# DanielTakeshi/gym-cloth

Hardware: AMD Instinct MI355X
Metric: cloth substeps/sec (25x25 grid, batched envs) (higher is better)
Workload: dtype f32

## Files before the change

### gym_cloth_amd/csrc/episode_loop.hpp

```cpp
#pragma once

#include "cloth_common.hpp"
#include "phase_strain.hpp"
#include "phase_collide.hpp"
#include "cloth_metrics.hpp"

namespace clothhip {

template <typename T, int NT, int PPT, int TAB, bool REST_REG, int FUSED, int NS = 0>
__global__ __launch_bounds__(NT, (Variant{(int)sizeof(T), NT, PPT, TAB, REST_REG}.waves_per_eu())) void k_run_schedule(StepArgs<T> A) {
    static_assert((NS == 0 || NS == 25 || NS == 50) && (NS == 0 || FUSED != 3), "grid-specialised builds exist for 25x25 and 50x50 (stepper_variants.hpp: CLOTH_SPEC_*)");
    static constexpr Variant V{(int)sizeof(T), NT, PPT, TAB, REST_REG};
    extern __shared__ __attribute__((aligned(16))) unsigned char smem[];
    const int e = blockIdx.x + A.e0;
    const int tid = threadIdx.x;
    const int lane = tid & 63;
    const FusedArgs<T> *const Fp = A.fz;
    constexpr bool fused = FUSED != 0;
    constexpr bool with_tier2 = FUSED == 2;
    constexpr bool RELAXED = FUSED == 3;
    ClothSchedule sc;
    if (!fused) {
        sc = A.sched[e];
        if (!sc.active || sc.n_total <= 0) {
            if (tid == 0) A.executed[e] = 0;
            return;
        }
    } else {
        sc.n_up_end = sc.n_uprest_end = sc.n_pull_end = sc.n_griprest_end = sc.n_total = 0;
        sc.break_on_tear = 1; sc.active = 1; sc._pad = 0;
        sc.dz_up = sc.dx_pull = sc.dy_pull = sc.dz_pull = 0.0;
    }
    const int P = NS > 0 ? spec_p(NS) : A.P, Ppad = NS > 0 ? spec_ppad(NS) : A.Ppad, HT = NS > 0 ? spec_ht(NS, V) : A.HT;
    constexpr bool LEAN64 = V.lean64();
    const LdsLayout lay = lds_layout(V, Ppad, KA_SPAD(&A), HT, KA_CELLCOPY(&A));
    Pt<T> *cur = reinterpret_cast<Pt<T> *>(smem + lay.cur);
    uint32_t *hkey = reinterpret_cast<uint32_t *>(smem + lay.hkey);
    uint32_t *hco = reinterpret_cast<uint32_t *>(smem + lay.hco);
    uint16_t *memb = reinterpret_cast<uint16_t *>(smem + lay.memb);
    uint16_t *slot = reinterpret_cast<uint16_t *>(smem + lay.slot);
    int *misc = reinterpret_cast<int *>(smem + lay.misc);
    uint16_t *olist = reinterpret_cast<uint16_t *>(smem + lay.olist);
    uint16_t *alist_end = olist + (Ppad - 1);
    Pt<T> *cpos = reinterpret_cast<Pt<T> *>(smem + lay.cpos);
    const T *g_rest = A.rest + (size_t)e * A.rest_stride;
    const WEnt<T> *wtab = reinterpret_cast<const WEnt<T> *>(smem + lay.wtab);
    auto rest_at = [&](uint32_t i) -> T { return V.table_in_lds() ? wtab[i].rest : g_rest[i]; };
    const int pm = NS > 0 ? (PH_HOOKE | PH_COLLIDE | PH_PLANE | PH_STRAIN) : A.phase_mask;

    T pvx[PPT], pvy[PPT], pvz[PPT];
    constexpr bool LEAN = V.lean();
    constexpr bool GT_REG = sizeof(T) == 4 && !LEAN;
    constexpr bool REST_R = V.rest_in_registers();
    uint32_t gt[GT_REG ? PPT : 1][HK_SLOTS];
    T rr[REST_R ? PPT : 1][HK_SLOTS];
    uint32_t vm[(LEAN && !LEAN64) ? PPT : 1];
    const uint4 *const lstc = reinterpret_cast<const uint4 *>(smem + lay.lstc);
    auto lean_rest64 = [&](int sl, const uint4 &lw) -> T {
        const uint32_t wsel = sl < 4 ? lw.y : (sl < 8 ? lw.z : lw.w);
        const uint32_t off = (wsel >> (8 * (sl & 3))) & 0xFFu;
        const double base = (double)(lean_bend(sl) ? A.pal_bend : (lean_shear(sl) ? A.pal_shear : A.pal_struct));
        return (T)__longlong_as_double(__double_as_longlong(base) + (long long)off);
    };
    (void)lean_rest64; (void)lstc;
    uint32_t rc[RELAXED ? PPT : 1];
    constexpr bool LEAN_NATIVE = LEAN && !LEAN64 && V.lean_native_gather();
    static_assert(!LEAN_NATIVE || (2 * NS <= V.cur_front_pad_records() && 2 * 27 <= V.cur_front_pad_records()), "the records in front of `cur` must cover the stencil's reach (two rows)");
    auto lean_entry = [&](int i, uint32_t vmq, int sl) -> uint32_t {
        const bool ok = ((vmq >> sl) & 1u) != 0u;
        return (uint32_t)(ok ? i + lean_off(sl, KA_N(&A)) : i) | (ok ? HK_VALID : 0u) | (sl < HK_SLOTS / 2 ? HK_ASB : 0u) |
               (lean_bend(sl) ? HK_BEND : 0u);
    };
    auto lean_rest = [&](int sl) -> T {
        if constexpr (NS > 0 && sizeof(T) == 4)
            return (T)(lean_bend(sl) ? spec_pal(NS, 2) : (lean_shear(sl) ? spec_pal(NS, 1) : spec_pal(NS, 0)));
        else return lean_bend(sl) ? A.pal_bend : (lean_shear(sl) ? A.pal_shear : A.pal_struct);
    };
    {
        const T *gp = A.pos + (size_t)e * 3 * Ppad, *gq = A.prev + (size_t)e * 3 * Ppad;
        const uint8_t *gc = A.cnt + (size_t)e * Ppad;
        if constexpr (V.cur_front_pad_records() > 0) {
            static_assert(V.cur_front_pad_records() <= NT, "one thread per record in front of `cur`");
            if (tid < V.cur_front_pad_records()) cur[tid - V.cur_front_pad_records()] = Pt<T>{(T)0, (T)0, (T)0, (T)0};
        }
        for (int i = tid; i < Ppad; i += NT)
            cur[i] = Pt<T>{gp[i], gp[Ppad + i], gp[2 * Ppad + i], w_make<T>(gc[i])};
#pragma unroll
        for (int q = 0; q < PPT; q++) {
            const int i = tid + q * NT;
            const bool ok = i < P;
            pvx[q] = ok ? gq[i] : (T)0; pvy[q] = ok ? gq[Ppad + i] : (T)0; pvz[q] = ok ? gq[2 * Ppad + i] : (T)0;
            if (LEAN64) { }
            else if (LEAN) { const int r_ = i / KA_N(&A); vm[(LEAN && !LEAN64) ? q : 0] = ok ? lean_valid_mask(r_, i - r_ * KA_N(&A), KA_N(&A)) : 0u; if (RELAXED) rc[RELAXED ? q : 0] = (uint32_t)r_ | ((uint32_t)(i - r_ * KA_N(&A)) << 8); }
            else
#pragma unroll
            for (int sl = 0; sl < HK_SLOTS; sl++) {
                const uint32_t g0 = ok ? A.gather[sl * Ppad + i] : 0u;
                if (GT_REG) gt[GT_REG ? q : 0][sl] = g0;
                if (REST_R) rr[REST_R ? q : 0][sl] = g_rest[(g0 >> HK_POS_SHIFT) & HK_POS_MASK];
            }
        }
    }
    auto init_lds = [&](int tear_flag, const uint32_t *s_ent, const T *s_rest) {
        if (V.table_in_lds() && s_ent != nullptr) {
            WEnt<T> *d0 = reinterpret_cast<WEnt<T> *>(smem + lay.wtab);
            for (int i = tid; i < KA_SPAD(&A); i += NT) { WEnt<T> w_; w_.ab = s_ent[i]; w_.rest = s_rest[i]; d0[i] = w_; }
        }
        for (int h = tid; h < HT; h += NT) { hkey[h] = KEY_EMPTY; hco[h] = 0; }
        if (tid == 0) { misc[0] = tear_flag; misc[1] = 0; misc[2] = 0; misc[3] = 0; misc[4] = 0; misc[5] = 0; misc[6] = 0; misc[10] = 0x7fffffff; misc[11] = -1; misc[12] = 0; misc[13] = 0; misc[14] = 0; misc[20] = 0; misc[21] = 0; misc[22] = 0; misc[23] = 0; }
    };
    if (tid == 0) misc[15] = 0;
    init_lds(A.tear[e], A.wt_ent, g_rest);
    if (LEAN64) {
        uint4 *d_ = reinterpret_cast<uint4 *>(smem + lay.lstc);
        for (int i = tid; i < Ppad; i += NT) d_[i] = A.lstc[i];
    }
    uint16_t *pslot = reinterpret_cast<uint16_t *>(smem + lay.pslot);
    if (V.has_point_slots()) {
        for (int i = tid; i < Ppad; i += NT) {
            const int r_ = i / KA_N(&A);
            const uint32_t vmi = i < P ? lean_valid_mask(r_, i - r_ * KA_N(&A), KA_N(&A)) : 0u;
#pragma unroll
            for (int sl = 0; sl < HK_SLOTS / 2; sl++)
                pslot[sl * Ppad + i] = ((vmi >> sl) & 1u) ? (uint16_t)((A.gather[__popc(vmi & ((1u << sl) - 1u)) * Ppad + i] >> HK_POS_SHIFT) & HK_POS_MASK) : (uint16_t)0;
        }
    }
    __syncthreads();

    int st_windows = 0, st_passes = 0, st_commits = 0;
#ifdef CLOTHHIP_TPH_LDS
    const TphLds tph{reinterpret_cast<unsigned long long *>(smem + lay.tphs), tid == 0};
    if (tid < 12) tph.base[tid] = 0ull;
    unsigned long long tlast = 0, tstart = 0;
#else
    unsigned long long tph[12] = {0, 0, 0, 0, 0, 0, 0, 0, 0, 0, 0, 0}, tlast = 0, tstart = 0;
#endif
    asm volatile("s_memtime %0\n\ts_waitcnt lgkmcnt(0)" : "=s"(tstart)::"memory");
#ifdef CLOTHHIP_DIAG_PLACEMENT
    const unsigned long long diag_t0_ = __builtin_amdgcn_s_memrealtime();
#endif
#ifdef CLOTHHIP_PHASE_STAMPS
    const bool timing = (pm & PH_TIME) != 0;
#else
    constexpr bool timing = false;
#endif
#ifdef CLOTHHIP_SWEEP_STAMPS
    constexpr bool SWEEP_TIMED = true;
#else
    constexpr bool SWEEP_TIMED = false;
#endif
#if !defined(CLOTHHIP_SWEEP_STAMPS) && !defined(CLOTHHIP_CELL_COUNTERS)
    constexpr bool SWEEP_LEAN = true;
#else
    constexpr bool SWEEP_LEAN = false;
#endif
    constexpr bool SWEEP_AHEAD = V.sweep_read_ahead();
    (void)SWEEP_AHEAD;
#if defined(CLOTHHIP_PHASE_STAMPS) || defined(CLOTHHIP_CELL_COUNTERS)
    constexpr bool SWEEP_STATS = true;
#else
    constexpr bool SWEEP_STATS = false;
#endif
#define TSTAMP(slot_)                                                          \
    if (timing) {                                                              \
        unsigned long long tn_;                                                \
        __builtin_amdgcn_sched_barrier(0);                                     \
        asm volatile("s_memtime %0\n\ts_waitcnt lgkmcnt(0)" : "=s"(tn_)::"memory"); \
        __builtin_amdgcn_sched_barrier(0);                                     \
        tph[slot_] += tn_ - tlast; tlast = tn_;                                \
    }
    if (timing) { asm volatile("s_memtime %0\n\ts_waitcnt lgkmcnt(0)" : "=s"(tlast)::"memory"); }

    enum { OP_SCHED = 0, OP_ACTION, OP_RESET_COND, OP_RESET_PULL, OP_RESET_SETTLE, OP_RESET_END };
    EpState *const eps = reinterpret_cast<EpState *>(smem + lay.eps);
    auto account = [&](int op_, int n_sub) {
        const int cls = op_ == OP_ACTION ? 0 : ((op_ == OP_RESET_PULL || op_ == OP_RESET_COND) ? 1 : (op_ == OP_RESET_SETTLE ? 2 : 3));
        const uint64_t now_ = __builtin_amdgcn_s_memrealtime();
        eps->ticks[cls] += now_ - eps->t_mark; eps->t_mark = now_; eps->subs[cls] += (uint32_t)n_sub;
    };
    if (fused) {
        if (tid == 0) {
            eps->t_slot = 0; eps->rp = -1; eps->n_resets = 0; eps->chain_ok = 1; eps->rs_pulls = 0; eps->reset_mark = 0;
            eps->ep_steps = Fp->num_steps[e]; eps->ep_done = Fp->done[e] ? 1 : 0; eps->done_total = 0; eps->stop = 0;
            misc[7] = 0;
            eps->t_mark = __builtin_amdgcn_s_memrealtime();
            for (int q = 0; q < 4; q++) { eps->ticks[q] = 0; eps->subs[q] = 0; }
            eps->last_cov = __longlong_as_double(0x7ff8000000000000LL); eps->n_ran = 0;
            eps->swap = Fp->policy_arg != nullptr ? Fp->policy_arg[e] : 0; eps->choice = 0;
            if (Fp->resume != nullptr && Fp->resume[e].valid) {
                const EpResume *rs_ = Fp->resume + e;
                const EpState &o = rs_->eps;
                eps->rp = o.rp; eps->chain_ok = o.chain_ok; eps->rs_pulls = o.rs_pulls; eps->ep_steps = o.ep_steps;
                eps->ep_done = o.ep_done; eps->op = o.op; eps->n_grab = o.n_grab; eps->iters_pull = o.iters_pull;
                eps->decode_err = o.decode_err; eps->side = o.side; eps->pull = o.pull; eps->choice = o.choice; eps->swap = o.swap;
                eps->act[0] = o.act[0]; eps->act[1] = o.act[1]; eps->act[2] = o.act[2]; eps->act[3] = o.act[3];
                if (o.rp >= 0 && Fp->resets != nullptr) Fp->resets[(size_t)e * Fp->n_scripts] = rs_->rr;
                if constexpr (with_tier2)
                    if (Fp->expert != 0 && o.rp < 0 && rs_->it >= 0) { double *lp = Fp->labels + 4 * (size_t)e; for (int q = 0; q < 4; q++) lp[q] = Fp->resume_labelled ? rs_->label[q] : __longlong_as_double(-1LL); }
            }
        }
        __syncthreads();
    }
    int resume_it = -1, resume_done = 0;
    if (FUSED) {
        if (Fp->resume != nullptr && Fp->resume[e].valid) {
            const EpResume *rs_ = Fp->resume + e;
            resume_it = rs_->it; resume_done = rs_->done_partial;
            if (resume_it >= 0) sc = rs_->sc;
        }
        __syncthreads();
        if (tid == 0 && Fp->resume != nullptr) Fp->resume[e].valid = 0;
    }
    if (FUSED) {
        if (tid == 0) {
            eps->t_launch = __builtin_amdgcn_s_memrealtime();
            eps->t_deadline = Fp->budget_ticks != 0 ? eps->t_launch + Fp->budget_ticks : ~0ull;
        }
    }
    int done_nf = 0;
    for (;;) {
        bool do_run = true;
        const bool resumed_run = FUSED && resume_it >= 0;
        if (fused && resumed_run) {
            sc.n_up_end = __builtin_amdgcn_readfirstlane(sc.n_up_end);
            sc.n_uprest_end = __builtin_amdgcn_readfirstlane(sc.n_uprest_end);
            sc.n_pull_end = __builtin_amdgcn_readfirstlane(sc.n_pull_end);
            sc.n_griprest_end = __builtin_amdgcn_readfirstlane(sc.n_griprest_end);
            sc.n_total = __builtin_amdgcn_readfirstlane(sc.n_total);
            sc.break_on_tear = __builtin_amdgcn_readfirstlane(sc.break_on_tear);
        }
        if (fused && !resumed_run) {
#include "episode_plan.inc.hpp"
        }
        int done = resumed_run ? resume_done : 0;
        int it_next = -1;
        {
        auto uni = [](T v) -> T {
            if constexpr (sizeof(T) == 4) return __int_as_float(__builtin_amdgcn_readfirstlane(__float_as_int((float)v)));
            else return __hiloint2double(__builtin_amdgcn_readfirstlane(__double2hiint((double)v)), __builtin_amdgcn_readfirstlane(__double2loint((double)v)));
        };
        const T dz_up = uni((T)sc.dz_up), dxp = uni((T)sc.dx_pull), dyp = uni((T)sc.dy_pull), dzp = uni((T)sc.dz_pull);
        const bool sliced = FUSED && Fp->budget_ticks != 0 && Fp->resume != nullptr;
        const int n_up_end_ = __builtin_amdgcn_readfirstlane(sc.n_up_end);
        const int n_uprest_end_ = __builtin_amdgcn_readfirstlane(sc.n_uprest_end);
        const int n_pull_end_ = __builtin_amdgcn_readfirstlane(sc.n_pull_end);
        const int n_griprest_end_ = __builtin_amdgcn_readfirstlane(sc.n_griprest_end);
        const int n_total_ = __builtin_amdgcn_readfirstlane(sc.n_total);
        const int break_on_tear_ = __builtin_amdgcn_readfirstlane(sc.break_on_tear);
        const int it0_ = __builtin_amdgcn_readfirstlane(resumed_run ? resume_it : 0);
    const int tid_outer_ = tid;
#ifdef CLOTHHIP_CELL_COUNTERS
    bool frozen_prev_ = false; (void)frozen_prev_;
#endif
    for (int it = it0_; it < n_total_; it++) {
        int tid = tid_outer_;
        if (LEAN || sizeof(T) == 8 || NT >= 512) asm volatile("" : "+v"(tid));
        const int lane = tid & 63;
        KArgsC<T> *Ak_ = (KArgsC<T> *)__builtin_amdgcn_kernarg_segment_ptr();

#include "substep_pull.inc.hpp"
        TSTAMP(0)
#include "substep_hooke_verlet.inc.hpp"
        TSTAMP(1)
#include "substep_collision.inc.hpp"
#include "substep_plane.inc.hpp"
        if (FUSED && sliced) {
            if (tid == 0) misc[7] = (__builtin_amdgcn_s_memrealtime() >= eps->t_deadline) ? 1 : 0;
        }
        __syncthreads();

        TSTAMP(7)
#include "substep_strain.inc.hpp"
        if (timing) { asm volatile("s_memtime %0\n\ts_waitcnt lgkmcnt(0)" : "=s"(tlast)::"memory"); }
        done++;
        if (break_on_tear_ && misc[0]) break;
        if (FUSED && sliced && misc[7] && it + 1 < n_total_) { it_next = it + 1; break; }
    }
        }
        resume_it = -1;
        if (!fused) { done_nf = done; break; }
#include "episode_finish.inc.hpp"
    }
    const int done = fused ? eps->done_total : done_nf;

#undef TSTAMP
    {
        __syncthreads();
        T *gp = A.pos + (size_t)e * 3 * Ppad, *gq = A.prev + (size_t)e * 3 * Ppad;
        uint8_t *gc = A.cnt + (size_t)e * Ppad;
        for (int i = tid; i < Ppad; i += NT) {
            const Pt<T> c = cur[i];
            gp[i] = c.x; gp[Ppad + i] = c.y; gp[2 * Ppad + i] = c.z; gc[i] = (uint8_t)w_cnt(c.w);
        }
#pragma unroll
        for (int q = 0; q < PPT; q++) {
            const int i = tid + q * NT;
            if (i < P) { gq[i] = pvx[q]; gq[Ppad + i] = pvy[q]; gq[2 * Ppad + i] = pvz[q]; }
        }
        if (tid == 0 && fused) {
            Fp->num_steps[e] = eps->ep_steps; Fp->done[e] = (uint8_t)eps->ep_done;
            if (Fp->summary != nullptr) {
                double *sm_ = Fp->summary + 4 * (size_t)e;
                sm_[0] = (double)eps->n_ran; sm_[1] = eps->ep_done ? 1.0 : 0.0; sm_[2] = eps->last_cov; sm_[3] = (double)eps->subs[0];
            }
            if (Fp->op_ticks != nullptr) {
                eps->ticks[3] += __builtin_amdgcn_s_memrealtime() - eps->t_mark;
                for (int q = 0; q < 4; q++) { Fp->op_ticks[8 * e + q] = eps->ticks[q]; Fp->op_ticks[8 * e + 4 + q] = eps->subs[q]; }
            }
        }
        if (tid == 0) {
            A.tear[e] = misc[0]; A.executed[e] = done;
            if (A.stats) {
                A.stats[16 * e] = misc[15]; A.stats[16 * e + 1] = st_windows; A.stats[16 * e + 2] = st_passes; A.stats[16 * e + 3] = st_commits;
                for (int q = 0; q < 12; q++) A.stats[16 * e + 4 + q] = (int)((unsigned long long)tph[q] >> 6);
#ifndef CLOTHHIP_PHASE_STAMPS
                unsigned long long tend;
                asm volatile("s_memtime %0\n\ts_waitcnt lgkmcnt(0)" : "=s"(tend)::"memory");
                A.stats[16 * e + 15] = (int)((tend - tstart) >> 10);
#endif
#ifdef CLOTHHIP_DIAG_PLACEMENT
                unsigned hw_, xcc_;
                asm volatile("s_getreg_b32 %0, hwreg(HW_REG_HW_ID)" : "=s"(hw_));
                asm volatile("s_getreg_b32 %0, hwreg(HW_REG_XCC_ID)" : "=s"(xcc_));
                A.stats[16 * e + 12] = (int)xcc_; A.stats[16 * e + 13] = (int)hw_;
                A.stats[16 * e + 14] = (int)(diag_t0_ & 0x7fffffffull); A.stats[16 * e + 11] = (int)(__builtin_amdgcn_s_memrealtime() & 0x7fffffffull);
#endif
            }
        }
    }
}

}
```

### gym_cloth_amd/csrc/phase_strain.hpp

```cpp
#pragma once

#include "cloth_common.hpp"

namespace clothhip {

template <typename T, bool LDS_TAB, bool TIMED, bool STATS, bool TIC>
__device__ __forceinline__ int strain_sweep(Pt<T> *cur, const WEnt<T> *wt, const uint32_t *g_ent, const T *g_rest,
                                            const unsigned long long *g_dep, int w0, int w_end,
                                            int nW, int rshift, const DevConsts<T> &k, int lane, int &st_windows, int &st_passes, int &st_commits,
                                            TphT tph, unsigned long long fmask = 0ull) {
    constexpr int PF = LDS_TAB ? 1 : 3;
    constexpr int PD = sizeof(T) == 4 ? 1 : 2;
    static_assert(PF + 1 <= WT_PAD_WINDOWS && PD + 1 <= WT_PAD_WINDOWS, "the table is padded by the read-ahead distance");
    int tear = 0;
    DevConsts<T> kl = k;
    asm volatile("" : "+v"(kl.c11), "+v"(kl.tear_thresh));
    constexpr bool tic = TIC;
    const T INF_ = sizeof(T) == 4 ? (T)__builtin_huge_valf() : (T)__builtin_huge_val();
    uint32_t eab[PF + 1]; T erest[PF + 1];
    unsigned long long edep[PD + 1];
    auto load = [&](int wi, uint32_t &ab_, T &r_) {
        if (LDS_TAB) { const WEnt<T> e_ = wt[wi * 64 + lane]; ab_ = e_.ab; r_ = e_.rest; }
        else { const uint32_t ix = (uint32_t)(wi * 64 + lane); ab_ = g_ent[ix]; r_ = g_rest[ix]; }
    };
#pragma unroll
    for (int j = 0; j <= PD; j++) edep[j] = g_dep[(uint32_t)((w0 + j) * 64 + lane)];
#pragma unroll
    for (int j = 0; j <= PF; j++) load(w0 + j, eab[j], erest[j]);
    struct __attribute__((aligned(16))) P3 { T x, y, z; };
    int w = w0;
    if (w > w_end) return tear;
#ifdef CLOTHHIP_CELL_COUNTERS
    int corr_end_ = w0 - 1;
#endif
    constexpr bool NEXT_AHEAD = sizeof(T) == 4;
    Pt<T> NA, NB;
    int an = (int)(eab[0] & WT_IDX_MASK), bn = (int)__builtin_amdgcn_ubfe(eab[0], WT_IDX_BITS, WT_IDX_BITS);
    NA = cur[an]; NB = cur[bn];
    do {
        const uint32_t ab = eab[0];
        const T rest = erest[0];
        const unsigned long long dep = edep[0];
#pragma unroll
        for (int j = 0; j < PF; j++) { eab[j] = eab[j + 1]; erest[j] = erest[j + 1]; }
#pragma unroll
        for (int j = 0; j < PD; j++) edep[j] = edep[j + 1];
        load(w + PF + 1, eab[PF], erest[PF]);
        edep[PD] = g_dep[(uint32_t)((w + PD + 1) * 64 + lane)];
        const int a = an, b = bn;
        P3 *const pa = reinterpret_cast<P3 *>(cur + a), *const pb = reinterpret_cast<P3 *>(cur + b);
        T ax, ay, az, bx, by, bz;
        uint32_t ca, cb;
        ax = NA.x; ay = NA.y; az = NA.z; bx = NB.x; by = NB.y; bz = NB.z;
        ca = w_cnt(NA.w); cb = w_cnt(NB.w);
        an = (int)(eab[0] & WT_IDX_MASK); bn = (int)__builtin_amdgcn_ubfe(eab[0], WT_IDX_BITS, WT_IDX_BITS);
        if (NEXT_AHEAD) { NA = cur[an]; NB = cur[bn]; }
        bool dirty = !NEXT_AHEAD;
        const T t11 = rest * kl.c11;
        const T tlim = ((ca != 0) & (cb != 0)) ? INF_ : t11;
        const uint32_t dlo = (uint32_t)dep, dhi = (uint32_t)(dep >> 32);
        bool pl = true;
        constexpr bool V1 = true;
        T tl = tlim;
        T tl2 = tlim * tlim * ((T)1 - filt_slack<T>());
        unsigned long long plm = ~0ull;
        if (STATS) st_windows++;
#ifdef CLOTHHIP_CELL_COUNTERS
        if (w > corr_end_ && !((fmask >> (w & 63)) & 1ull)) tph[3] += 64;
#endif
        bool more;
        do {
            unsigned long long td0 = 0;
            if (TIMED) { asm volatile("s_memtime %0\n\ts_waitcnt lgkmcnt(0)" : "=s"(td0)::"memory"); }
            const T dx = ax - bx, dy = ay - by, dz = az - bz;
            const T len2 = sumsq<T>(dx, dy, dz);
            bool trig;
            T len;
            if constexpr (sizeof(T) == 4) {
                len = dev_sqrt<T>(len2);
                trig = len > (V1 ? tl : tlim);
            } else {
                trig = false; len = (T)0;
                if (len2 > (V1 ? tl2 : tlim * tlim * ((T)1 - filt_slack<T>()))) {
                    len = dev_sqrt<T>(len2);
                    trig = len > (V1 ? tl : tlim);
                }
            }
            const unsigned long long tb = V1 ? ballot64(trig) : ballot64(trig & pl);
            if (STATS) st_passes++;
            bool bad = false;
            if (tb) bad = ((dlo & (uint32_t)tb) | (dhi & (uint32_t)(tb >> 32))) != 0u;
            if (!tic) {
                const bool mine = pl & !bad;
                if (mine && !((ca != 0) & (cb != 0)) && dev_sqrt<T>(len2) > rest * kl.tear_thresh) tear = 1;
            }
            more = false;
            if (tb) {
                const int reach = w + ((int)((uint32_t)__builtin_amdgcn_readfirstlane((int)ab) >> WT_REACH_SHIFT) << rshift);
                w_end = reach > w_end ? reach : w_end;
#ifdef CLOTHHIP_CELL_COUNTERS
                corr_end_ = reach > corr_end_ ? reach : corr_end_;
#endif
                dirty = true;
                if (STATS) st_commits++;
                if (V1 ? (trig & !bad) : (trig & pl & !bad)) {
                    if (tic && len > rest * kl.tear_thresh) tear = 1;
                    const T ux = dev_div<T>(dx, len), uy = dev_div<T>(dy, len), uz = dev_div<T>(dz, len);
                    const T extra = len - t11;
                    const T wa = ca != 0 ? (T)0 : (cb != 0 ? (T)1 : (T)0.5);
                    const T wb = cb != 0 ? (T)0 : (ca != 0 ? (T)1 : (T)0.5);
                    const T ea = extra * wa, eb = extra * wb;
                    *pa = P3{mad<T>(-ux, ea, ax), mad<T>(-uy, ea, ay), mad<T>(-uz, ea, az)};
                    *pb = P3{mad<T>(ux, eb, bx), mad<T>(uy, eb, by), mad<T>(uz, eb, bz)};
                }
                pl = pl & bad;
                if (V1) { tl = pl ? tl : INF_; if (sizeof(T) == 8) tl2 = pl ? tl2 : INF_; plm &= ballot64(bad); more = plm != 0ull; }
                else more = ballot64(pl) != 0ull;
                if (TIMED) { unsigned long long td1; asm volatile("s_memtime %0\n\ts_waitcnt lgkmcnt(0)" : "=s"(td1)::"memory"); tph[11] += td1 - td0; }
                if (more) {
                    __builtin_amdgcn_wave_barrier();
                    const P3 na = *pa, nb = *pb;
                    ax = na.x; ay = na.y; az = na.z; bx = nb.x; by = nb.y; bz = nb.z;
                }
            } else if (TIMED) { unsigned long long td1; asm volatile("s_memtime %0\n\ts_waitcnt lgkmcnt(0)" : "=s"(td1)::"memory"); tph[10] += td1 - td0; tph[9] += 64; }
        } while (more);
        w++;
        if (dirty) { NA = cur[an]; NB = cur[bn]; }
    } while (w <= w_end);
    return tear;
}

template <typename T, bool LDS_TAB, bool STATS, bool AHEAD = true>
__device__ __forceinline__ int strain_sweep_lean(Pt<T> *cur, const WEnt<T> *wt, const uint32_t *g_ent, const T *g_rest,
                                                 const unsigned long long *g_dep, int w0, int w_end, int rshift, const DevConsts<T> &k,
                                                 int lane, int &st_windows, int &st_passes, int &st_commits) {
    static_assert(WT_PAD_WINDOWS >= 3, "the entry stream reads two windows ahead, the particle reads one");
    int tear = 0;
    T c11 = k.c11, tth = k.tear_thresh;
    asm volatile("" : "+v"(c11), "+v"(tth));
    const T INF_ = sizeof(T) == 4 ? (T)__builtin_huge_valf() : (T)__builtin_huge_val();
    struct __attribute__((aligned(16))) P3 { T x, y, z; };
    struct Set { uint32_t ab; T rest; unsigned long long dep; int a, b; Pt<T> A, B; };
    auto load = [&](int wi, Set &s) {
        const uint32_t ix = (uint32_t)(wi * 64 + lane);
        if (LDS_TAB) { const WEnt<T> e_ = wt[ix]; s.ab = e_.ab; s.rest = e_.rest; }
        else { s.ab = g_ent[ix]; s.rest = g_rest[ix]; }
        s.dep = g_dep[ix];
    };
    auto decode_read = [&](Set &s) {
        s.a = (int)(s.ab & WT_IDX_MASK); s.b = (int)__builtin_amdgcn_ubfe(s.ab, WT_IDX_BITS, WT_IDX_BITS);
        s.A = cur[s.a]; s.B = cur[s.b];
    };
    int w = w0;
    auto step = [&](Set &c, Set &n) {
        if (AHEAD) decode_read(n);
        else decode_read(c);
        T ax = c.A.x, ay = c.A.y, az = c.A.z, bx = c.B.x, by = c.B.y, bz = c.B.z;
        T dx = ax - bx, dy = ay - by, dz = az - bz;
        T len2 = sumsq<T>(dx, dy, dz);
        const T t11 = c.rest * c11;
        T len = (T)0; bool trig;
        if constexpr (sizeof(T) == 4) { len = dev_sqrt<T>(len2); trig = len > t11; }
        else trig = len2 > t11 * t11 * ((T)1 - filt_slack<T>());
        if (STATS) { st_windows++; st_passes++; }
        if (ballot64(trig) != 0ull) {
            const uint32_t ca = w_cnt(c.A.w), cb = w_cnt(c.B.w);
#if defined(CLOTHHIP_MUTATE) && CLOTHHIP_MUTATE == 4
            T tl = t11;
#else
            T tl = ((ca != 0) & (cb != 0)) ? INF_ : t11;
#endif
            T tl2 = tl * tl * ((T)1 - filt_slack<T>());
            auto test = [&]() {
                if constexpr (sizeof(T) == 4) { trig = len > tl; }
                else { trig = false; if (len2 > tl2) { len = dev_sqrt<T>(len2); trig = len > tl; } }
            };
            test();
            unsigned long long tb = ballot64(trig);
            if (tb) {
                P3 *const pa = reinterpret_cast<P3 *>(cur + c.a), *const pb = reinterpret_cast<P3 *>(cur + c.b);
                const uint32_t dlo = (uint32_t)c.dep, dhi = (uint32_t)(c.dep >> 32);
                const int reach = w + ((int)((uint32_t)__builtin_amdgcn_readfirstlane((int)c.ab) >> WT_REACH_SHIFT) << rshift);
                w_end = reach > w_end ? reach : w_end;
                bool pl = true;
                unsigned long long plm = ~0ull;
                for (;;) {
#if defined(CLOTHHIP_MUTATE) && CLOTHHIP_MUTATE == 3
                    const unsigned long long tb2_ = tb & (tb - 1ull);
                    const bool bad = (((dlo & (uint32_t)tb) | (dhi & (uint32_t)(tb >> 32))) != 0u) && !(tb2_ != 0ull && lane == __ffsll((long long)tb2_) - 1);
#else
                    const bool bad = ((dlo & (uint32_t)tb) | (dhi & (uint32_t)(tb >> 32))) != 0u;
#endif
                    if (STATS) st_commits++;
                    if (trig & !bad) {
                        if (len > c.rest * tth) tear = 1;
                        const T ux = dev_div<T>(dx, len), uy = dev_div<T>(dy, len), uz = dev_div<T>(dz, len);
                        const T extra = len - t11;
                        const T wa = ca != 0 ? (T)0 : (cb != 0 ? (T)1 : (T)0.5);
                        const T wb = cb != 0 ? (T)0 : (ca != 0 ? (T)1 : (T)0.5);
                        const T ea = extra * wa, eb = extra * wb;
                        *pa = P3{mad<T>(-ux, ea, ax), mad<T>(-uy, ea, ay), mad<T>(-uz, ea, az)};
                        *pb = P3{mad<T>(ux, eb, bx), mad<T>(uy, eb, by), mad<T>(uz, eb, bz)};
                    }
                    pl = pl & bad;
                    tl = pl ? tl : INF_; if (sizeof(T) == 8) tl2 = pl ? tl2 : INF_;
                    plm &= ballot64(bad);
                    if (__builtin_expect(plm == 0ull, 0)) break;
                    __builtin_amdgcn_wave_barrier();
                    const P3 na = *pa, nb = *pb;
                    ax = na.x; ay = na.y; az = na.z; bx = nb.x; by = nb.y; bz = nb.z;
                    dx = ax - bx; dy = ay - by; dz = az - bz;
                    len2 = sumsq<T>(dx, dy, dz);
                    if constexpr (sizeof(T) == 4) len = dev_sqrt<T>(len2);
                    test();
                    tb = ballot64(trig);
                    if (STATS) st_passes++;
                    if (__builtin_expect(tb == 0ull, 0)) break;
                }
                if (AHEAD) { n.A = cur[n.a]; n.B = cur[n.b]; }
            }
        }
        load(w + 2, c);
    };
    Set S0, S1;
    load(w, S0); load(w + 1, S1);
    if (AHEAD) decode_read(S0);
    for (;;) {
        step(S0, S1);
        if (++w > w_end) break;
        step(S1, S0);
        if (++w > w_end) break;
    }
    return tear;
}

}
```

### gym_cloth_amd/csrc/stepper_traits.hpp

```cpp
#pragma once

namespace clothhip {

constexpr int
    TAB_LEAN_6 = -3,
    TAB_LEAN_5 = -2,
    TAB_LEAN_4 = -1,
    TAB_STREAM = 0,
    TAB_LDS = 1,
    TAB_LDS_SLOTS = 2,
    TAB_LARGE_1 = 3,
    TAB_LARGE_2 = 4;
constexpr int LDS_TABLE_NONE = 0, LDS_TABLE = 1, LDS_TABLE_SLOTS = 2;

struct Variant {
    int tsz, nt, ppt, tab;
    bool rest_reg;

    constexpr bool operator==(const Variant &o) const { return tsz == o.tsz && nt == o.nt && ppt == o.ppt && tab == o.tab && rest_reg == o.rest_reg; }
    constexpr bool lean() const { return rest_reg && (tsz == 4 ? tab != TAB_LDS : tab == TAB_STREAM); }
    constexpr bool lean64() const { return lean() && tsz == 8; }
    constexpr bool rest_in_registers() const { return rest_reg && !lean(); }
    constexpr bool table_in_lds() const { return tab == TAB_LDS || tab == TAB_LDS_SLOTS; }
    constexpr int lds_table_mode() const { return tab == TAB_LDS_SLOTS ? LDS_TABLE_SLOTS : (table_in_lds() ? LDS_TABLE : LDS_TABLE_NONE); }
    constexpr bool has_point_slots() const { return tab == TAB_LDS_SLOTS; }
    constexpr bool sweep_read_ahead() const { return tab >= TAB_LDS; }
    constexpr int built_for_cloths_per_cu() const {
        if (lean() && tsz == 4) return tab == TAB_LARGE_1 ? 1 : ((tab == TAB_LDS_SLOTS || tab == TAB_LARGE_2) ? 2 : 3 + (TAB_STREAM - tab));
        return nt * ppt <= 1024 ? 2 : 1;
    }
    constexpr int waves_per_eu() const { return built_for_cloths_per_cu() * (nt / 64) / 4; }
    constexpr bool hull_as_indices() const { return tab == TAB_LARGE_2 || tab <= TAB_LEAN_5 || (tsz == 8 && nt * ppt > 1024) || nt * ppt >= 4096; }
    constexpr bool collide_two_visits_per_trip() const { return tab <= TAB_LEAN_6; }
    constexpr bool lean_native_gather() const { return tsz == 4 && tab == TAB_LDS_SLOTS; }
    constexpr int cur_front_pad_records() const { return lean_native_gather() ? 64 : 0; }
    constexpr bool spec_ht_fitted() const { return tab == TAB_LARGE_2; }
    constexpr bool spec_has_cell_copy() const { return tab > TAB_LEAN_5; }
};

constexpr Variant lean_four_wave(int r) { return Variant{4, 256, 3, r >= 4 ? TAB_STREAM - (r - 3) : TAB_STREAM, true}; }

}
```

### gym_cloth_amd/csrc/substep_strain.inc.hpp

```cpp
        if constexpr (RELAXED) {
            CLOTH_PHASE_ARGS()
            static_assert(!RELAXED || LEAN, "the relaxed-order companion exists for the LEAN arithmetic (stencil from the grid position, palette rest lengths)");
            int tear_ = 0;
#pragma unroll 1
            for (int col = 0; col < 12; col++) {
                const int kind = col >> 1, par = col & 1;
#pragma unroll
                for (int q = 0; q < PPT; q++) {
                    const int i = tid + q * NT;
                    const int r_ = (int)(rc[RELAXED ? q : 0] & 0xFFu), c_ = (int)(rc[RELAXED ? q : 0] >> 8);
                    const int key = (kind == 1 || kind == 5) ? c_ : r_;
                    const bool on = i < P && ((vm[(LEAN && !LEAN64) ? q : 0] >> kind) & 1u) && (((kind >= 4 ? key >> 1 : key) & 1) == par);
                    if (on) {
                        const int j = i + (kind == 0 ? -Ak_->N : kind == 1 ? -1 : kind == 2 ? -Ak_->N - 1 : kind == 3 ? -Ak_->N + 1 : kind == 4 ? -2 * Ak_->N : -2);
                        const Pt<T> a_ = cur[j], b_ = cur[i];
                        const uint32_t ca = w_cnt(a_.w), cb = w_cnt(b_.w);
                        const T rest = kind >= 4 ? Ak_->pal_bend : (kind >= 2 ? Ak_->pal_shear : Ak_->pal_struct);
                        const T dx = a_.x - b_.x, dy = a_.y - b_.y, dz = a_.z - b_.z;
                        const T len = fastnorm<T>(dx, dy, dz);
                        if (!((ca != 0) & (cb != 0))) {
                            if (len > rest * k.tear_thresh) tear_ = 1;
                            const T t11 = rest * k.c11;
                            if (len > t11) {
                                const T ux = dev_div<T>(dx, len), uy = dev_div<T>(dy, len), uz = dev_div<T>(dz, len);
                                const T extra = len - t11;
                                const T wa = ca != 0 ? (T)0 : (cb != 0 ? (T)1 : (T)0.5), wb = cb != 0 ? (T)0 : (ca != 0 ? (T)1 : (T)0.5);
                                const T ea = extra * wa, eb = extra * wb;
                                if (ca == 0) cur[j] = Pt<T>{mad<T>(-ux, ea, a_.x), mad<T>(-uy, ea, a_.y), mad<T>(-uz, ea, a_.z), a_.w};
                                if (cb == 0) cur[i] = Pt<T>{mad<T>(ux, eb, b_.x), mad<T>(uy, eb, b_.y), mad<T>(uz, eb, b_.z), b_.w};
                            }
                        }
                    }
                }
                __syncthreads();
            }
            if (__any(tear_) && lane == 0) misc[0] = 1;
            __syncthreads();
        } else
        if (pm & PH_STRAIN) {
            CLOTH_PHASE_ARGS()
            {
                int nact = 0, pmin = 0x7fffffff, pmax = -1;
#pragma unroll
                for (int q = 0; q < PPT; q++) {
                    if (tid + q * NT < P) {
                        const Pt<T> me = cur[tid + q * NT];
                        const uint32_t cme_ = w_cnt(me.w);
                        uint32_t gl[HK_SLOTS / 2];
                        int iq_ = tid + q * NT; uint4 lw_ = uint4{0u, 0u, 0u, 0u}; if constexpr (LEAN64) lw_ = lstc[iq_]; uint32_t vq_ = LEAN64 ? lw_.x : vm[(LEAN && !LEAN64) ? q : 0];
                        if (LEAN) asm volatile("" : "+v"(iq_), "+v"(vq_));
#pragma unroll
                        for (int sl = 0; sl < HK_SLOTS / 2; sl++)
                            gl[sl] = LEAN_NATIVE ? 0u : LEAN ? lean_entry(iq_, vq_, sl) : (GT_REG ? gt[GT_REG ? q : 0][sl] : Ak_->gather[sl * Ppad + tid + q * NT]);
                        constexpr int PP_AHEAD = 2;
                        Pt<T> nbq[PP_AHEAD];
#pragma unroll
                        for (int sl = 0; sl < PP_AHEAD; sl++) {
                            if constexpr (LEAN_NATIVE) nbq[sl] = cur[iq_ + lean_off(sl, KA_N(Ak_))];
                            else {
                            uint32_t g = gl[sl];
                            asm volatile("" : "+v"(g));
                            gl[sl] = g;
                            nbq[sl] = cur[g & HK_NBR_MASK];
                            }
                        }
                        uint32_t cand = 0u;
                        T l2s[HK_SLOTS / 2];
#pragma unroll
                        for (int sl = 0; sl < HK_SLOTS / 2; sl++) {
                            const uint32_t g = gl[sl];
                            const Pt<T> nb = nbq[sl % PP_AHEAD];
                            if (sl + PP_AHEAD < HK_SLOTS / 2) {
                                if constexpr (LEAN_NATIVE) nbq[sl % PP_AHEAD] = cur[iq_ + lean_off(sl + PP_AHEAD, KA_N(Ak_))];
                                else {
                                uint32_t gn = gl[sl + PP_AHEAD];
                                asm volatile("" : "+v"(gn));
                                gl[sl + PP_AHEAD] = gn;
                                nbq[sl % PP_AHEAD] = cur[gn & HK_NBR_MASK];
                                }
                            }
                            __builtin_amdgcn_sched_barrier(0);
                            T r = LEAN64 ? lean_rest64(sl, lw_) : LEAN ? lean_rest(sl) : (REST_R ? rr[REST_R ? q : 0][sl] : rest_at((g >> HK_POS_SHIFT) & HK_POS_MASK));
                            asm volatile("" : "+v"(r));
                            const T dx = nb.x - me.x, dy = nb.y - me.y, dz = nb.z - me.z;
                            const T len2 = sumsq<T>(dx, dy, dz);
                            l2s[sl] = len2;
                            const T t11 = r * k.c11, tt = r * k.tear_thresh;
                            const T tmin = t11 < tt ? t11 : tt;
#if defined(CLOTHHIP_MUTATE) && CLOTHHIP_MUTATE == 4
                            const bool pre = (LEAN_NATIVE ? (vq_ & (1u << sl)) != 0u : (g & (HK_VALID | HK_ASB)) == (HK_VALID | HK_ASB)) &
                                             (len2 > tmin * tmin * ((T)1 - filt_slack<T>()));
#else
                            const bool pre = (LEAN_NATIVE ? (vq_ & (1u << sl)) != 0u : (g & (HK_VALID | HK_ASB)) == (HK_VALID | HK_ASB)) &
                                             !((cme_ != 0) & (w_cnt(nb.w) != 0)) &
                                             (len2 > tmin * tmin * ((T)1 - filt_slack<T>()));
#endif
                            cand |= pre ? (1u << sl) : 0u;
                        }
                        if (cand) {
#pragma unroll
                            for (int sl = 0; sl < HK_SLOTS / 2; sl++) {
                                if (cand & (1u << sl)) {
                                    const uint32_t pos_ = V.has_point_slots() ? (uint32_t)pslot[sl * Ppad + iq_] : ((LEAN ? Ak_->gather[__popc(vq_ & ((1u << sl) - 1u)) * Ppad + iq_] : gl[sl])
                                                           >> HK_POS_SHIFT) & HK_POS_MASK;
                                    T r = LEAN64 ? lean_rest64(sl, lw_) : LEAN ? lean_rest(sl) : (REST_R ? rr[REST_R ? q : 0][sl] : rest_at(pos_));
                                    asm volatile("" : "+v"(r));
                                    const T len2 = l2s[sl];
                                    const T t11 = r * k.c11, tt = r * k.tear_thresh;
                                    const T tmin = t11 < tt ? t11 : tt;
                                    bool flag = len2 > tmin * tmin * ((T)1 + filt_slack<T>());
                                    if (!flag) { const T len = dev_sqrt<T>(len2); flag = len > t11 || len > tt; }
                                    if (flag) { nact++; pmin = (int)pos_ < pmin ? (int)pos_ : pmin; pmax = (int)pos_ > pmax ? (int)pos_ : pmax; }
#ifdef CLOTHHIP_CELL_COUNTERS
                                    if (flag) atomicOr(&misc[13 + (((int)pos_ >> 6) >> 5 & 1)], 1 << (((int)pos_ >> 6) & 31));
#endif
                                }
                            }
                        }
                    }
                }
                if (__any(nact)) {
                    const int min_ = __builtin_amdgcn_readlane(wave_incl_min(pmin), 63);
                    const int max_ = -__builtin_amdgcn_readlane(wave_incl_min(-pmax), 63);
                    if (lane == 0) { misc[1] = 1; atomicMin(&misc[10], min_); atomicMax(&misc[11], max_); }
                }
            }
            __syncthreads();
            TSTAMP(8)
#ifdef CLOTHHIP_CELL_COUNTERS
            int swept_ = 0;
#endif
            if (tid < 64 && (misc[1] || (pm & PH_NOSKIP))) {
                __builtin_amdgcn_s_setprio(3);
                const bool all_ = (pm & PH_NOSKIP) != 0;
                const int w0 = __builtin_amdgcn_readfirstlane(all_ ? 0 : (misc[10] >> 6));
                const int w1 = __builtin_amdgcn_readfirstlane(all_ ? KA_NW(Ak_) - 1 : (misc[11] >> 6));
                if (lane == 0) misc[15]++;
                const bool tic = __builtin_amdgcn_readfirstlane(!(k.tear_thresh < k.c11) ? 1 : 0) != 0;
#ifdef CLOTHHIP_CELL_COUNTERS
                const unsigned long long fmask_ = (unsigned long long)(uint32_t)misc[13] | ((unsigned long long)(uint32_t)misc[14] << 32);
                swept_ = 1;
#else
                const unsigned long long fmask_ = 0ull;
#endif
                const int tear = tic ? (SWEEP_LEAN ? strain_sweep_lean<T, V.table_in_lds(), SWEEP_STATS, SWEEP_AHEAD>(cur, wtab, Ak_->wt_ent, g_rest, Ak_->wt_dep, w0, w1, KA_RSHIFT(Ak_), k,
                                                                                                  lane, st_windows, st_passes, st_commits)
                                                   : strain_sweep<T, V.table_in_lds(), SWEEP_TIMED, SWEEP_STATS, true>(cur, wtab, Ak_->wt_ent, g_rest, Ak_->wt_dep, w0, w1, Ak_->nW, KA_RSHIFT(Ak_), k,
                                                                                                 lane, st_windows, st_passes, st_commits, tph, fmask_))
                                     : strain_sweep<T, V.table_in_lds(), SWEEP_TIMED, SWEEP_STATS, false>(cur, wtab, Ak_->wt_ent, g_rest, Ak_->wt_dep, w0, w1, Ak_->nW, KA_RSHIFT(Ak_), k,
                                                                                                  lane, st_windows, st_passes, st_commits, tph, fmask_);
                if (__any(tear) && lane == 0) misc[0] = 1;
                if (lane == 0) { misc[1] = 0; misc[10] = 0x7fffffff; misc[11] = -1; }
#ifdef CLOTHHIP_CELL_COUNTERS
                if (lane == 0) { misc[13] = 0; misc[14] = 0; }
#endif
                __builtin_amdgcn_s_setprio(0);
            }
            __syncthreads();
#ifndef CLOTHHIP_SWEEP_STAMPS
            TSTAMP(9)
#endif
#ifdef CLOTHHIP_CELL_COUNTERS
            if (tid < 64) {
                const bool frozen_ = mode != 1 && misc[12] == 0 && !swept_ && k.one_m_fric == (T)0;
                tph[1] += frozen_ ? 64 : 0; tph[2] += misc[16] == 0 ? 64 : 0;
                frozen_prev_ = frozen_;
            }
            __syncthreads();
            if (tid == 0) { misc[12] = 0; misc[16] = 0; }
#endif
        }
```

Measured before the change: 17.60 million.

## Start strain sweep speculatively on wave 0 while other waves run prepass

For the 512-thread, 2-points-per-thread lean-native variant, wave 0 no longer waits at a barrier for the strain prepass. It sweeps windows in small speculative grants while the other seven waves redistribute the prepass work and signal completion through an LDS counter. Once the prepass is done, the sweep extends or skips ahead to the flagged window range. This hides the prepass latency behind the serial sweep. The cost is extra sweep work on windows that may be clean, spin-polling with sleep, fewer threads doing the prepass, and a timeout fallback that reports a stats flag.

Measured after the change: 17.91 million (median of 6 runs). 1.02x the previous value.

```diff
diff --git a/gym_cloth_amd/csrc/episode_loop.hpp b/gym_cloth_amd/csrc/episode_loop.hpp
--- a/gym_cloth_amd/csrc/episode_loop.hpp
+++ b/gym_cloth_amd/csrc/episode_loop.hpp
@@ -108,8 +108,10 @@
         }
         for (int h = tid; h < HT; h += NT) { hkey[h] = KEY_EMPTY; hco[h] = 0; }
         if (tid == 0) { misc[0] = tear_flag; misc[1] = 0; misc[2] = 0; misc[3] = 0; misc[4] = 0; misc[5] = 0; misc[6] = 0; misc[10] = 0x7fffffff; misc[11] = -1; misc[12] = 0; misc[13] = 0; misc[14] = 0; misc[20] = 0; misc[21] = 0; misc[22] = 0; misc[23] = 0; }
+        if constexpr (V.sweep_starts_early()) { if (tid == 0) misc[17] = 0; }
     };
     if (tid == 0) misc[15] = 0;
+    if constexpr (V.sweep_starts_early()) { if (tid == 0 && A.stats) A.stats[16 * e + 4] = 0; }
     init_lds(A.tear[e], A.wt_ent, g_rest);
     if (LEAN64) {
         uint4 *d_ = reinterpret_cast<uint4 *>(smem + lay.lstc);
@@ -153,6 +155,11 @@
     constexpr bool SWEEP_LEAN = true;
 #else
     constexpr bool SWEEP_LEAN = false;
+#endif
+#if defined(CLOTHHIP_PHASE_STAMPS)
+    constexpr bool SWEEP_EARLY = false;
+#else
+    constexpr bool SWEEP_EARLY = SWEEP_LEAN && V.sweep_starts_early();
 #endif
     constexpr bool SWEEP_AHEAD = V.sweep_read_ahead();
     (void)SWEEP_AHEAD;
@@ -312,7 +319,7 @@
             A.tear[e] = misc[0]; A.executed[e] = done;
             if (A.stats) {
                 A.stats[16 * e] = misc[15]; A.stats[16 * e + 1] = st_windows; A.stats[16 * e + 2] = st_passes; A.stats[16 * e + 3] = st_commits;
-                for (int q = 0; q < 12; q++) A.stats[16 * e + 4 + q] = (int)((unsigned long long)tph[q] >> 6);
+                for (int q = SWEEP_EARLY ? 1 : 0; q < 12; q++) A.stats[16 * e + 4 + q] = (int)((unsigned long long)tph[q] >> 6);
 #ifndef CLOTHHIP_PHASE_STAMPS
                 unsigned long long tend;
                 asm volatile("s_memtime %0\n\ts_waitcnt lgkmcnt(0)" : "=s"(tend)::"memory");
diff --git a/gym_cloth_amd/csrc/phase_strain.hpp b/gym_cloth_amd/csrc/phase_strain.hpp
--- a/gym_cloth_amd/csrc/phase_strain.hpp
+++ b/gym_cloth_amd/csrc/phase_strain.hpp
@@ -130,10 +130,12 @@
     return tear;
 }
 
-template <typename T, bool LDS_TAB, bool STATS, bool AHEAD = true>
+constexpr int EARLY_GRANT = 4, EARLY_WAIT_POLLS = 4096;
+template <typename T, bool LDS_TAB, bool STATS, bool AHEAD = true, bool EARLY = false>
 __device__ __forceinline__ int strain_sweep_lean(Pt<T> *cur, const WEnt<T> *wt, const uint32_t *g_ent, const T *g_rest,
                                                  const unsigned long long *g_dep, int w0, int w_end, int rshift, const DevConsts<T> &k,
-                                                 int lane, int &st_windows, int &st_passes, int &st_commits) {
+                                                 int lane, int &st_windows, int &st_passes, int &st_commits,
+                                                 bool early = false, int *misc = nullptr, int nW = 0) {
     static_assert(WT_PAD_WINDOWS >= 3, "the entry stream reads two windows ahead, the particle reads one");
     int tear = 0;
     T c11 = k.c11, tth = k.tear_thresh;
@@ -223,13 +225,49 @@
         load(w + 2, c);
     };
     Set S0, S1;
-    load(w, S0); load(w + 1, S1);
-    if (AHEAD) decode_read(S0);
-    for (;;) {
-        step(S0, S1);
-        if (++w > w_end) break;
-        step(S1, S0);
-        if (++w > w_end) break;
+    if constexpr (!EARLY) {
+        load(w, S0); load(w + 1, S1);
+        if (AHEAD) decode_read(S0);
+        for (;;) {
+            step(S0, S1);
+            if (++w > w_end) break;
+            step(S1, S0);
+            if (++w > w_end) break;
+        }
+    } else {
+        constexpr int NPRE = 7;
+        auto peek = [&](int i) -> int { return __builtin_amdgcn_readfirstlane(__hip_atomic_load(&misc[i], __ATOMIC_RELAXED, __HIP_MEMORY_SCOPE_WORKGROUP)); };
+        auto done = [&]() -> bool { return __builtin_amdgcn_readfirstlane(__hip_atomic_load(&misc[17], __ATOMIC_ACQUIRE, __HIP_MEMORY_SCOPE_WORKGROUP)) >= NPRE; };
+        (void)peek;
+        bool known = !early;
+        if (early) w_end = (EARLY_GRANT < nW ? EARLY_GRANT : nW) - 1;
+        for (;;) {
+            load(w, S0); load(w + 1, S1);
+            if (AHEAD) decode_read(S0);
+            for (;;) {
+                step(S0, S1);
+                if (++w > w_end) break;
+                step(S1, S0);
+                if (++w > w_end) break;
+            }
+            if (known) break;
+            if (!done()) {
+                if (w < nW) { w_end = (w + EARLY_GRANT < nW ? w + EARLY_GRANT : nW) - 1; continue; }
+                int polls = 0;
+                bool d_;
+                do { __builtin_amdgcn_s_sleep(8); d_ = done(); } while (!d_ && ++polls < EARLY_WAIT_POLLS);
+                if (!d_) { tear |= 2; break; }
+            }
+            known = true;
+#if !(defined(CLOTHHIP_MUTATE) && CLOTHHIP_MUTATE == 5)
+            if (peek(1) != 0) {
+                const int wf = peek(10) >> 6, wl = peek(11) >> 6;
+                w_end = wl > w_end ? wl : w_end;
+                w = wf > w ? wf : w;
+            }
+#endif
+            if (w > w_end) break;
+        }
     }
     return tear;
 }
diff --git a/gym_cloth_amd/csrc/stepper_traits.hpp b/gym_cloth_amd/csrc/stepper_traits.hpp
--- a/gym_cloth_amd/csrc/stepper_traits.hpp
+++ b/gym_cloth_amd/csrc/stepper_traits.hpp
@@ -34,6 +34,8 @@
     constexpr bool collide_two_visits_per_trip() const { return tab <= TAB_LEAN_6; }
     constexpr bool lean_native_gather() const { return tsz == 4 && tab == TAB_LDS_SLOTS; }
     constexpr int cur_front_pad_records() const { return lean_native_gather() ? 64 : 0; }
+    constexpr bool sweep_starts_early() const { return lean_native_gather() && nt == 512 && ppt == 2; }
+    constexpr int early_prepass_threads() const { return nt - 64; }
     constexpr bool spec_ht_fitted() const { return tab == TAB_LARGE_2; }
     constexpr bool spec_has_cell_copy() const { return tab > TAB_LEAN_5; }
 };
diff --git a/gym_cloth_amd/csrc/substep_strain.inc.hpp b/gym_cloth_amd/csrc/substep_strain.inc.hpp
--- a/gym_cloth_amd/csrc/substep_strain.inc.hpp
+++ b/gym_cloth_amd/csrc/substep_strain.inc.hpp
@@ -39,86 +39,19 @@
         } else
         if (pm & PH_STRAIN) {
             CLOTH_PHASE_ARGS()
+#ifdef CLOTHHIP_CELL_COUNTERS
+            int swept_ = 0;
+#endif
+            if constexpr (SWEEP_EARLY) {
+#include "substep_strain_early.inc.hpp"
+            } else {
             {
                 int nact = 0, pmin = 0x7fffffff, pmax = -1;
-#pragma unroll
-                for (int q = 0; q < PPT; q++) {
-                    if (tid + q * NT < P) {
-                        const Pt<T> me = cur[tid + q * NT];
-                        const uint32_t cme_ = w_cnt(me.w);
-                        uint32_t gl[HK_SLOTS / 2];
-                        int iq_ = tid + q * NT; uint4 lw_ = uint4{0u, 0u, 0u, 0u}; if constexpr (LEAN64) lw_ = lstc[iq_]; uint32_t vq_ = LEAN64 ? lw_.x : vm[(LEAN && !LEAN64) ? q : 0];
-                        if (LEAN) asm volatile("" : "+v"(iq_), "+v"(vq_));
-#pragma unroll
-                        for (int sl = 0; sl < HK_SLOTS / 2; sl++)
-                            gl[sl] = LEAN_NATIVE ? 0u : LEAN ? lean_entry(iq_, vq_, sl) : (GT_REG ? gt[GT_REG ? q : 0][sl] : Ak_->gather[sl * Ppad + tid + q * NT]);
-                        constexpr int PP_AHEAD = 2;
-                        Pt<T> nbq[PP_AHEAD];
-#pragma unroll
-                        for (int sl = 0; sl < PP_AHEAD; sl++) {
-                            if constexpr (LEAN_NATIVE) nbq[sl] = cur[iq_ + lean_off(sl, KA_N(Ak_))];
-                            else {
-                            uint32_t g = gl[sl];
-                            asm volatile("" : "+v"(g));
-                            gl[sl] = g;
-                            nbq[sl] = cur[g & HK_NBR_MASK];
-                            }
-                        }
-                        uint32_t cand = 0u;
-                        T l2s[HK_SLOTS / 2];
-#pragma unroll
-                        for (int sl = 0; sl < HK_SLOTS / 2; sl++) {
-                            const uint32_t g = gl[sl];
-                            const Pt<T> nb = nbq[sl % PP_AHEAD];
-                            if (sl + PP_AHEAD < HK_SLOTS / 2) {
-                                if constexpr (LEAN_NATIVE) nbq[sl % PP_AHEAD] = cur[iq_ + lean_off(sl + PP_AHEAD, KA_N(Ak_))];
-                                else {
-                                uint32_t gn = gl[sl + PP_AHEAD];
-                                asm volatile("" : "+v"(gn));
-                                gl[sl + PP_AHEAD] = gn;
-                                nbq[sl % PP_AHEAD] = cur[gn & HK_NBR_MASK];
-                                }
-                            }
-                            __builtin_amdgcn_sched_barrier(0);
-                            T r = LEAN64 ? lean_rest64(sl, lw_) : LEAN ? lean_rest(sl) : (REST_R ? rr[REST_R ? q : 0][sl] : rest_at((g >> HK_POS_SHIFT) & HK_POS_MASK));
-                            asm volatile("" : "+v"(r));
-                            const T dx = nb.x - me.x, dy = nb.y - me.y, dz = nb.z - me.z;
-                            const T len2 = sumsq<T>(dx, dy, dz);
-                            l2s[sl] = len2;
-                            const T t11 = r * k.c11, tt = r * k.tear_thresh;
-                            const T tmin = t11 < tt ? t11 : tt;
-#if defined(CLOTHHIP_MUTATE) && CLOTHHIP_MUTATE == 4
-                            const bool pre = (LEAN_NATIVE ? (vq_ & (1u << sl)) != 0u : (g & (HK_VALID | HK_ASB)) == (HK_VALID | HK_ASB)) &
-                                             (len2 > tmin * tmin * ((T)1 - filt_slack<T>()));
-#else
-                            const bool pre = (LEAN_NATIVE ? (vq_ & (1u << sl)) != 0u : (g & (HK_VALID | HK_ASB)) == (HK_VALID | HK_ASB)) &
-                                             !((cme_ != 0) & (w_cnt(nb.w) != 0)) &
-                                             (len2 > tmin * tmin * ((T)1 - filt_slack<T>()));
-#endif
-                            cand |= pre ? (1u << sl) : 0u;
-                        }
-                        if (cand) {
-#pragma unroll
-                            for (int sl = 0; sl < HK_SLOTS / 2; sl++) {
-                                if (cand & (1u << sl)) {
-                                    const uint32_t pos_ = V.has_point_slots() ? (uint32_t)pslot[sl * Ppad + iq_] : ((LEAN ? Ak_->gather[__popc(vq_ & ((1u << sl) - 1u)) * Ppad + iq_] : gl[sl])
-                                                           >> HK_POS_SHIFT) & HK_POS_MASK;
-                                    T r = LEAN64 ? lean_rest64(sl, lw_) : LEAN ? lean_rest(sl) : (REST_R ? rr[REST_R ? q : 0][sl] : rest_at(pos_));
-                                    asm volatile("" : "+v"(r));
-                                    const T len2 = l2s[sl];
-                                    const T t11 = r * k.c11, tt = r * k.tear_thresh;
-                                    const T tmin = t11 < tt ? t11 : tt;
-                                    bool flag = len2 > tmin * tmin * ((T)1 + filt_slack<T>());
-                                    if (!flag) { const T len = dev_sqrt<T>(len2); flag = len > t11 || len > tt; }
-                                    if (flag) { nact++; pmin = (int)pos_ < pmin ? (int)pos_ : pmin; pmax = (int)pos_ > pmax ? (int)pos_ : pmax; }
-#ifdef CLOTHHIP_CELL_COUNTERS
-                                    if (flag) atomicOr(&misc[13 + (((int)pos_ >> 6) >> 5 & 1)], 1 << (((int)pos_ >> 6) & 31));
-#endif
-                                }
-                            }
-                        }
-                    }
-                }
+#define PP_IDX_(q_) tid + (q_) * NT
+#define PP_MASK_(q_)
+#include "substep_strain_prepass.inc.hpp"
+#undef PP_IDX_
+#undef PP_MASK_
                 if (__any(nact)) {
                     const int min_ = __builtin_amdgcn_readlane(wave_incl_min(pmin), 63);
                     const int max_ = -__builtin_amdgcn_readlane(wave_incl_min(-pmax), 63);
@@ -127,9 +60,6 @@
             }
             __syncthreads();
             TSTAMP(8)
-#ifdef CLOTHHIP_CELL_COUNTERS
-            int swept_ = 0;
-#endif
             if (tid < 64 && (misc[1] || (pm & PH_NOSKIP))) {
                 __builtin_amdgcn_s_setprio(3);
                 const bool all_ = (pm & PH_NOSKIP) != 0;
@@ -140,6 +70,7 @@
 #ifdef CLOTHHIP_CELL_COUNTERS
                 const unsigned long long fmask_ = (unsigned long long)(uint32_t)misc[13] | ((unsigned long long)(uint32_t)misc[14] << 32);
                 swept_ = 1;
+                if (w0 == (e & 63)) tph[0] += 1ull << 22;
 #else
                 const unsigned long long fmask_ = 0ull;
 #endif
@@ -157,6 +88,7 @@
                 __builtin_amdgcn_s_setprio(0);
             }
             __syncthreads();
+            }
 #ifndef CLOTHHIP_SWEEP_STAMPS
             TSTAMP(9)
 #endif
diff --git a/gym_cloth_amd/csrc/substep_strain_early.inc.hpp b/gym_cloth_amd/csrc/substep_strain_early.inc.hpp
--- /dev/null
+++ b/gym_cloth_amd/csrc/substep_strain_early.inc.hpp
@@ -0,0 +1,36 @@
+            constexpr int EARLY_NT = V.early_prepass_threads();
+            const bool tic = __builtin_amdgcn_readfirstlane(!(k.tear_thresh < k.c11) ? 1 : 0) != 0;
+            const bool early_ = tic && __builtin_amdgcn_readfirstlane((!(pm & PH_NOSKIP) && P <= 2 * EARLY_NT) ? 1 : 0) != 0;
+            if (!(early_ && tid < 64)) {
+                int nact = 0, pmin = 0x7fffffff, pmax = -1;
+#define PP_IDX_(q_) (early_ ? (tid - 64) + (q_) * EARLY_NT : tid + (q_) * NT)
+#define PP_MASK_(q_) if (early_) { const int r_ = iq_ / KA_N(Ak_); vq_ = lean_valid_mask(r_, iq_ - r_ * KA_N(Ak_), KA_N(Ak_)); }
+#include "substep_strain_prepass.inc.hpp"
+#undef PP_IDX_
+#undef PP_MASK_
+                if (__any(nact)) {
+                    const int min_ = __builtin_amdgcn_readlane(wave_incl_min(pmin), 63);
+                    const int max_ = -__builtin_amdgcn_readlane(wave_incl_min(-pmax), 63);
+                    if (lane == 0) { misc[1] = 1; atomicMin(&misc[10], min_); atomicMax(&misc[11], max_); }
+                }
+                if (early_ && lane == 0) __hip_atomic_fetch_add(&misc[17], 1, __ATOMIC_RELEASE, __HIP_MEMORY_SCOPE_WORKGROUP);
+            }
+            if (!early_) __syncthreads();
+            if (tid < 64 && (early_ || misc[1] || (pm & PH_NOSKIP))) {
+                __builtin_amdgcn_s_setprio(3);
+                const bool all_ = (pm & PH_NOSKIP) != 0;
+                const int w0 = early_ ? 0 : __builtin_amdgcn_readfirstlane(all_ ? 0 : (misc[10] >> 6));
+                const int w1 = early_ ? -1 : __builtin_amdgcn_readfirstlane(all_ ? KA_NW(Ak_) - 1 : (misc[11] >> 6));
+                int tear = tic ? strain_sweep_lean<T, V.table_in_lds(), SWEEP_STATS, SWEEP_AHEAD, true>(cur, wtab, Ak_->wt_ent, g_rest, Ak_->wt_dep, w0, w1, KA_RSHIFT(Ak_), k,
+                                                                                                  lane, st_windows, st_passes, st_commits, early_, misc, KA_NW(Ak_))
+                               : strain_sweep<T, V.table_in_lds(), SWEEP_TIMED, SWEEP_STATS, false>(cur, wtab, Ak_->wt_ent, g_rest, Ak_->wt_dep, w0, w1, Ak_->nW, KA_RSHIFT(Ak_), k,
+                                                                                                    lane, st_windows, st_passes, st_commits, tph, 0ull);
+                if (tear & 2) { if (lane == 0 && A.stats) atomicAdd(&A.stats[16 * e + 4], 1); }
+                tear &= 1;
+                if (__any(tear) && lane == 0) misc[0] = 1;
+                if (early_) { if (lane == 0 && __hip_atomic_load(&misc[1], __ATOMIC_RELAXED, __HIP_MEMORY_SCOPE_WORKGROUP) != 0) misc[15]++; }
+                else if (lane == 0) { misc[15]++; misc[1] = 0; misc[10] = 0x7fffffff; misc[11] = -1; }
+                __builtin_amdgcn_s_setprio(0);
+            }
+            __syncthreads();
+            if (early_ && tid == NT - 1) { misc[1] = 0; misc[10] = 0x7fffffff; misc[11] = -1; misc[17] = 0; }
diff --git a/gym_cloth_amd/csrc/substep_strain_prepass.inc.hpp b/gym_cloth_amd/csrc/substep_strain_prepass.inc.hpp
--- /dev/null
+++ b/gym_cloth_amd/csrc/substep_strain_prepass.inc.hpp
@@ -0,0 +1,79 @@
+#pragma unroll
+                for (int q = 0; q < PPT; q++) {
+                    if (PP_IDX_(q) < P) {
+                        const Pt<T> me = cur[PP_IDX_(q)];
+                        const uint32_t cme_ = w_cnt(me.w);
+                        uint32_t gl[HK_SLOTS / 2];
+                        int iq_ = PP_IDX_(q); uint4 lw_ = uint4{0u, 0u, 0u, 0u}; if constexpr (LEAN64) lw_ = lstc[iq_]; uint32_t vq_ = LEAN64 ? lw_.x : vm[(LEAN && !LEAN64) ? q : 0];
+                        PP_MASK_(q)
+                        if (LEAN) asm volatile("" : "+v"(iq_), "+v"(vq_));
+#pragma unroll
+                        for (int sl = 0; sl < HK_SLOTS / 2; sl++)
+                            gl[sl] = LEAN_NATIVE ? 0u : LEAN ? lean_entry(iq_, vq_, sl) : (GT_REG ? gt[GT_REG ? q : 0][sl] : Ak_->gather[sl * Ppad + PP_IDX_(q)]);
+                        constexpr int PP_AHEAD = 2;
+                        Pt<T> nbq[PP_AHEAD];
+#pragma unroll
+                        for (int sl = 0; sl < PP_AHEAD; sl++) {
+                            if constexpr (LEAN_NATIVE) nbq[sl] = cur[iq_ + lean_off(sl, KA_N(Ak_))];
+                            else {
+                            uint32_t g = gl[sl];
+                            asm volatile("" : "+v"(g));
+                            gl[sl] = g;
+                            nbq[sl] = cur[g & HK_NBR_MASK];
+                            }
+                        }
+                        uint32_t cand = 0u;
+                        T l2s[HK_SLOTS / 2];
+#pragma unroll
+                        for (int sl = 0; sl < HK_SLOTS / 2; sl++) {
+                            const uint32_t g = gl[sl];
+                            const Pt<T> nb = nbq[sl % PP_AHEAD];
+                            if (sl + PP_AHEAD < HK_SLOTS / 2) {
+                                if constexpr (LEAN_NATIVE) nbq[sl % PP_AHEAD] = cur[iq_ + lean_off(sl + PP_AHEAD, KA_N(Ak_))];
+                                else {
+                                uint32_t gn = gl[sl + PP_AHEAD];
+                                asm volatile("" : "+v"(gn));
+                                gl[sl + PP_AHEAD] = gn;
+                                nbq[sl % PP_AHEAD] = cur[gn & HK_NBR_MASK];
+                                }
+                            }
+                            __builtin_amdgcn_sched_barrier(0);
+                            T r = LEAN64 ? lean_rest64(sl, lw_) : LEAN ? lean_rest(sl) : (REST_R ? rr[REST_R ? q : 0][sl] : rest_at((g >> HK_POS_SHIFT) & HK_POS_MASK));
+                            asm volatile("" : "+v"(r));
+                            const T dx = nb.x - me.x, dy = nb.y - me.y, dz = nb.z - me.z;
+                            const T len2 = sumsq<T>(dx, dy, dz);
+                            l2s[sl] = len2;
+                            const T t11 = r * k.c11, tt = r * k.tear_thresh;
+                            const T tmin = t11 < tt ? t11 : tt;
+#if defined(CLOTHHIP_MUTATE) && CLOTHHIP_MUTATE == 4
+                            const bool pre = (LEAN_NATIVE ? (vq_ & (1u << sl)) != 0u : (g & (HK_VALID | HK_ASB)) == (HK_VALID | HK_ASB)) &
+                                             (len2 > tmin * tmin * ((T)1 - filt_slack<T>()));
+#else
+                            const bool pre = (LEAN_NATIVE ? (vq_ & (1u << sl)) != 0u : (g & (HK_VALID | HK_ASB)) == (HK_VALID | HK_ASB)) &
+                                             !((cme_ != 0) & (w_cnt(nb.w) != 0)) &
+                                             (len2 > tmin * tmin * ((T)1 - filt_slack<T>()));
+#endif
+                            cand |= pre ? (1u << sl) : 0u;
+                        }
+                        if (cand) {
+#pragma unroll
+                            for (int sl = 0; sl < HK_SLOTS / 2; sl++) {
+                                if (cand & (1u << sl)) {
+                                    const uint32_t pos_ = V.has_point_slots() ? (uint32_t)pslot[sl * Ppad + iq_] : ((LEAN ? Ak_->gather[__popc(vq_ & ((1u << sl) - 1u)) * Ppad + iq_] : gl[sl])
+                                                           >> HK_POS_SHIFT) & HK_POS_MASK;
+                                    T r = LEAN64 ? lean_rest64(sl, lw_) : LEAN ? lean_rest(sl) : (REST_R ? rr[REST_R ? q : 0][sl] : rest_at(pos_));
+                                    asm volatile("" : "+v"(r));
+                                    const T len2 = l2s[sl];
+                                    const T t11 = r * k.c11, tt = r * k.tear_thresh;
+                                    const T tmin = t11 < tt ? t11 : tt;
+                                    bool flag = len2 > tmin * tmin * ((T)1 + filt_slack<T>());
+                                    if (!flag) { const T len = dev_sqrt<T>(len2); flag = len > t11 || len > tt; }
+                                    if (flag) { nact++; pmin = (int)pos_ < pmin ? (int)pos_ : pmin; pmax = (int)pos_ > pmax ? (int)pos_ : pmax; }
+#ifdef CLOTHHIP_CELL_COUNTERS
+                                    if (flag) atomicOr(&misc[13 + (((int)pos_ >> 6) >> 5 & 1)], 1 << (((int)pos_ >> 6) & 31));
+#endif
+                                }
+                            }
+                        }
+                    }
+                }
```
